# JoshuaQSH/FALCON-TTDforGNNs

Measured on NVIDIA B200. Metric: TT-EmbeddingBag rows/s fwd+bwd+SGD, higher is better.
Workload: dtype f32

## Files before the change

### falcon-ttdforgnns_b200/csrc/tt_rmma.cu

```cuda
#include <stdlib.h>

#include "common.cuh"

namespace ttg {

namespace {

constexpr int kThreads = 512;
constexpr int kWarps = kThreads / 32;
constexpr uint32_t kFull = 0xffffffffu;
constexpr int kCS = 20;

__device__ __forceinline__ uint32_t smem_u32(const void* p) { return (uint32_t)__cvta_generic_to_shared(p); }

__device__ __forceinline__ void mma_tf32(float (&c)[4], uint32_t a0, uint32_t a1, uint32_t a2, uint32_t a3,
                                         uint32_t b0, uint32_t b1) {
  asm("mma.sync.aligned.m16n8k8.row.col.f32.tf32.tf32.f32 {%0,%1,%2,%3}, {%4,%5,%6,%7}, {%8,%9}, "
      "{%0,%1,%2,%3};"
      : "+f"(c[0]), "+f"(c[1]), "+f"(c[2]), "+f"(c[3])
      : "r"(a0), "r"(a1), "r"(a2), "r"(a3), "r"(b0), "r"(b1));
}
__device__ __forceinline__ float lo_of(float x) {
  return x - __uint_as_float(__float_as_uint(x) & 0xffffe000u);
}
// ... 510 lines not shown
      const uint32_t grp = __shfl_sync(kFull, my_grp, 0);
      const uint32_t same = __ballot_sync(kFull, pos + (lane & 7) < re && my_grp == grp) & 0xffu;
      const int n = min(4, __ffs(~same) - 1);
      const bool group_ends = ((same >> n) & 1u) == 0;
      const bool more = pos + n < re;
      const uint32_t next_grp = __shfl_sync(kFull, my_grp, n);
      if (group_ends && more) prefetch_tr1<C>(a.tab, next_grp, lane);
      int i0r[4];
#pragma unroll
      for (int j = 0; j < 4; ++j) {
        const int v = __shfl_sync(kFull, my_i0, j);
        i0r[j] = (j < n) ? v : -1;
      }
      const int slot_pos = (pos - rs) & (kRing - 1);
      RM_PHASE(0);
      cp_async_wait<kRing / 4 - 1>();
      __syncwarp();
      RM_PHASE(1);
#ifdef TTG_R_TIMING
      if (pos == rs) RM_MARK(3);
#endif

      float g0[2][4];
#pragma unroll
      for (int nt = 0; nt < 2; ++nt)
#pragma unroll
        for (int e = 0; e < 4; ++e) g0[nt][e] = 0.f;
      {
        const float* pa = ring + ((slot_pos + rg) & (kRing - 1)) * RS;
        const float* pb = ring + ((slot_pos + rg + 2) & (kRing - 1)) * RS;
#pragma unroll
        for (int ks = 0; ks < 4; ++ks) {
          const float x0 = pa[xoff<C>(j0, col_k<C>(ks, 0, t))], x2 = pa[xoff<C>(j0, col_k<C>(ks, 1, t))];
          const float x1 = pb[xoff<C>(j0, col_k<C>(ks, 0, t))], x3 = pb[xoff<C>(j0, col_k<C>(ks, 1, t))];
          const uint32_t h0 = __float_as_uint(x0), h1 = __float_as_uint(x1), h2 = __float_as_uint(x2),
                         h3 = __float_as_uint(x3);
          if (TERMS == 3) {
            const uint32_t l0 = __float_as_uint(lo_of(x0)), l1 = __float_as_uint(lo_of(x1)),
                           l2 = __float_as_uint(lo_of(x2)), l3 = __float_as_uint(lo_of(x3));
#pragma unroll
            for (int nt = 0; nt < 2; ++nt) mma_tf32(g0[nt], l0, l1, l2, l3, bgh[ks][nt][0], bgh[ks][nt][1]);
#pragma unroll
            for (int nt = 0; nt < 2; ++nt) mma_tf32(g0[nt], h0, h1, h2, h3, bgl[ks][nt][0], bgl[ks][nt][1]);
          }
#pragma unroll
          for (int nt = 0; nt < 2; ++nt) mma_tf32(g0[nt], h0, h1, h2, h3, bgh[ks][nt][0], bgh[ks][nt][1]);
        }
      }
      RM_PHASE(2);
      if (group_ends && more) load_tr1_bwd<C, TERMS>(a.tab, next_grp, g, t, bgh, bgl);
      RM_PHASE(3);

#pragma unroll
      for (int ks = 0; ks < 2; ++ks) {
        const float* ce = c0s + ((i0r[2 * ks] < 0 ? a.c0_rows : i0r[2 * ks]) * 4 + t) * kCSB + g;
        const float* co = c0s + ((i0r[2 * ks + 1] < 0 ? a.c0_rows : i0r[2 * ks + 1]) * 4 + t) * kCSB + g;
        const float a0 = ce[0], a1 = ce[8], a2 = co[0], a3 = co[8];
        const uint32_t ah0 = __float_as_uint(a0), ah1 = __float_as_uint(a1), ah2 = __float_as_uint(a2),
                       ah3 = __float_as_uint(a3);
        const uint32_t al0 = __float_as_uint(lo_of(a0)), al1 = __float_as_uint(lo_of(a1)),
                       al2 = __float_as_uint(lo_of(a2)), al3 = __float_as_uint(lo_of(a3));
        const float* pe = ring + ((slot_pos + 2 * ks) & (kRing - 1)) * RS;
        const float* po = ring + ((slot_pos + 2 * ks + 1) & (kRing - 1)) * RS;
#pragma unroll
        for (int nt = 0; nt < 4; ++nt) {
          const float b0 = pe[xoff<C>(t, col_n<C>(nt, g))], b1 = po[xoff<C>(t, col_n<C>(nt, g))];
          if (TERMS == 3) {
            mma_tf32(s1[nt], al0, al1, al2, al3, __float_as_uint(b0), __float_as_uint(b1));
            mma_tf32(s1[nt], ah0, ah1, ah2, ah3, __float_as_uint(lo_of(b0)), __float_as_uint(lo_of(b1)));
          }
          mma_tf32(s1[nt], ah0, ah1, ah2, ah3, __float_as_uint(b0), __float_as_uint(b1));
        }
      }

      RM_PHASE(4);
      {
        int i0a = rg ? i0r[1] : i0r[0], i0b = rg ? i0r[3] : i0r[2];
        i0a = i0a < 0 ? a.c0_rows + warp : i0a;
        i0b = i0b < 0 ? a.c0_rows + warp : i0b;
        const int ra = i0a * 4 + j0, rb = i0b * 4 + j0;
        float* da = d0s + ra * 16;
        float* db = d0s + rb * 16;
        const int swa = d0_swizzle(ra), swb = d0_swizzle(rb);
        float* addr[8];
        float val[8];
#pragma unroll
        for (int nt = 0; nt < 2; ++nt)
#pragma unroll
          for (int e = 0; e < 2; ++e) {
            addr[4 * nt + e] = da + ((2 * t + 8 * nt + e) ^ swa);
            val[4 * nt + e] = g0[nt][e];
            addr[4 * nt + 2 + e] = db + ((2 * t + 8 * nt + e) ^ swb);
            val[4 * nt + 2 + e] = g0[nt][2 + e];
          }
        shared_add_batch<8>(addr, val);
      }

      RM_PHASE(5);
      ++chain;
      if (group_ends || chain == kChain) {
        float* dst = a.S1 + (size_t)grp * (16 * C);
#pragma unroll
        for (int nt = 0; nt < 4; ++nt) {
#pragma unroll
          for (int e = 0; e < 2; ++e) {
            const int c = col_n<C>(nt, 2 * t + e);
            if ((C % 8 == 0) || c < C) {
              float* d0 = dst + g * C + c;
              float* d1 = dst + (g + 8) * C + c;
              float v0 = s1[nt][e], v1 = s1[nt][2 + e];
              if (stored) {
                v0 += ld_dep_f32(d0);
                v1 += ld_dep_f32(d1);
              }
              *d0 = v0;
              *d1 = v1;
            }
          }
#pragma unroll
          for (int e = 0; e < 4; ++e) s1[nt][e] = 0.f;
        }
        stored = !group_ends;
        chain = 0;
      }
      __syncwarp();
      pos += n;
      RM_PHASE(6);
    }
    RM_PHASE_FLUSH;
    cp_async_wait<0>();
    __syncwarp();
  }
  }
  RM_MARK(4);
  __syncthreads();
  float* part = a.d0parts + (size_t)blockIdx.x * a.c0_rows * 64;
  for (int i = threadIdx.x; i < a.c0_rows * 64; i += kBT) part[i] = d0s[(i & ~15) + ((i & 15) ^ d0_swizzle(i >> 4))];
  RM_MARK(5);
}

constexpr int kCoresThreads = 512, kCoresWarps = kCoresThreads / 32;
constexpr int kCoresGB = 8;
constexpr int kCoresBufs = 3;
constexpr int kC2S = 24;

#ifdef TTG_R_TIMING
__device__ unsigned long long g_rc_marks[1024 * 6];
#define RC_MARK(i) \
  if (threadIdx.x == 0 && blockIdx.x < 1024) g_rc_marks[blockIdx.x * 6 + (i)] = gtime()
#else
#define RC_MARK(i)
#endif

template <int Q1, int Q2>
__global__ void __launch_bounds__(kCoresThreads, 1)
rm_cores_kernel(TTDev tt, const float* S1, const int32_t* cnt, float* __restrict__ dcore1, float* __restrict__ parts2,
                int dbg) {
  constexpr int C = Q1 * Q2, NR = 16 * Q1, IMG = 16 * C, R2 = 16, GB = kCoresGB;
  constexpr int KB = GB * Q2;
  constexpr int KSA = KB / 8;
  constexpr int MT = NR / 16;
  constexpr int NTB = KB / 8;
  constexpr int KSB = NR / 8;
  constexpr int BLK4 = GB * IMG / 4;
  static_assert(KB % 8 == 0 && NR % 16 == 0 && 2 * MT + NTB <= kCoresWarps, "tile shapes");
  extern __shared__ __align__(16) float sm[];
  const int p1 = tt.p[1], p2 = tt.p[2];
  const int nblk = (p2 + GB - 1) / GB;
  float* c2s = sm;
  float* sbuf = c2s + (size_t)nblk * KB * kC2S;
  __shared__ int32_t cnts[512 + kCoresGB];
  const int lane = threadIdx.x & 31, warp = threadIdx.x >> 5, g = lane >> 2, t = lane & 3;
  const int ti1 = blockIdx.x, table = ti1 / p1;
  const size_t h0 = (size_t)ti1 * p2;
  RC_MARK(0);
  pdl_trigger();
  {
    const float* core2 = tt.core[2] + (size_t)table * p2 * (R2 * Q2);
    constexpr int PER = kCoresThreads / (R2 * Q2);
    const int e = threadIdx.x % (R2 * Q2), k2 = e / Q2, j2 = e % Q2;
    if (threadIdx.x < PER * R2 * Q2)
      for (int i2 = threadIdx.x / (R2 * Q2); i2 < nblk * GB; i2 += PER)
        c2s[((size_t)i2 * Q2 + j2) * kC2S + k2] = (i2 < p2) ? __ldg(core2 + (size_t)i2 * (R2 * Q2) + e) : 0.f;
  }
  const bool role_a = warp < 2 * MT, role_b = !role_a && warp < 2 * MT + NTB;
  uint32_t ah[KSB][4], al[KSB][4];
  if (role_b) {
    const float* c1 = tt.core[1] + (size_t)ti1 * (NR * R2);
#pragma unroll
    for (int ks = 0; ks < KSB; ++ks) {
      const float v0 = __ldg(c1 + (t + 8 * ks) * R2 + g), v1 = __ldg(c1 + (t + 8 * ks) * R2 + g + 8);
      const float v2 = __ldg(c1 + (t + 4 + 8 * ks) * R2 + g), v3 = __ldg(c1 + (t + 4 + 8 * ks) * R2 + g + 8);
      ah[ks][0] = __float_as_uint(v0);
      ah[ks][1] = __float_as_uint(v1);
      ah[ks][2] = __float_as_uint(v2);
      ah[ks][3] = __float_as_uint(v3);
      al[ks][0] = __float_as_uint(lo_of(v0));
      al[ks][1] = __float_as_uint(lo_of(v1));
      al[ks][2] = __float_as_uint(lo_of(v2));
      al[ks][3] = __float_as_uint(lo_of(v3));
    }
  }
  RC_MARK(1);
  pdl_wait();
  RC_MARK(2);
  for (int i = threadIdx.x; i < nblk * GB; i += kCoresThreads) cnts[i] = (i < p2) ? ld_dep_s32(cnt + h0 + i) : 0;
  __syncthreads();
  RC_MARK(3);
  auto stage = [&](int blk) {
    if (blk < nblk && !(dbg & 2)) {
      float* dst = sbuf + (size_t)(blk % kCoresBufs) * (GB * IMG);
      const float* src = S1 + (h0 + (size_t)blk * GB) * IMG;
      for (int i = threadIdx.x; i < BLK4; i += kCoresThreads) {
        if (cnts[blk * GB + i / (IMG / 4)] > 0)
          cp_async16(dst + 4 * i, src + 4 * i);
        else
          *reinterpret_cast<float4*>(dst + 4 * i) = make_float4(0.f, 0.f, 0.f, 0.f);
      }
    }
    cp_async_commit();
  };
  const int mt = warp >> 1, nt = warp & 1;
  int offa[KSA][2];
#pragma unroll
  for (int ks = 0; ks < KSA; ++ks)
#pragma unroll
    for (int h = 0; h < 2; ++h) {
      const int kk = t + 4 * h + 8 * ks;
      offa[ks][h] = (kk / Q2) * IMG + (kk % Q2) + (g + 16 * mt) * Q2;
    }
  const int ntb = warp - 2 * MT;
  const int nnb = g + 8 * ntb, offb = (nnb / Q2) * IMG + (nnb % Q2) + t * Q2;
  float acc1[2][4] = {{0.f, 0.f, 0.f, 0.f}, {0.f, 0.f, 0.f, 0.f}};
  stage(0);
  stage(1);
  for (int blk = 0; blk < nblk; ++blk) {
    cp_async_wait<1>();
    __syncthreads();
#ifdef TTG_R_TIMING
    if (blk == 0) RC_MARK(4);
#endif
    stage(blk + 2);
    const float* sb = sbuf + (size_t)(blk % kCoresBufs) * (GB * IMG);
    if (dbg & 1) continue;
    if (role_a) {
      const float* cb = c2s + (size_t)blk * KB * kC2S + g + 8 * nt;
      float part[3][4] = {{0.f, 0.f, 0.f, 0.f}, {0.f, 0.f, 0.f, 0.f}, {0.f, 0.f, 0.f, 0.f}};
#pragma unroll
      for (int ks = 0; ks < KSA; ++ks) {
        const float a0 = sb[offa[ks][0]], a1 = sb[offa[ks][0] + 8 * Q2];
        const float a2 = sb[offa[ks][1]], a3 = sb[offa[ks][1] + 8 * Q2];
        const float b0 = cb[(t + 8 * ks) * kC2S], b1 = cb[(t + 4 + 8 * ks) * kC2S];
        mma_tf32(part[0], __float_as_uint(lo_of(a0)), __float_as_uint(lo_of(a1)), __float_as_uint(lo_of(a2)),
                 __float_as_uint(lo_of(a3)), __float_as_uint(b0), __float_as_uint(b1));
        mma_tf32(part[1], __float_as_uint(a0), __float_as_uint(a1), __float_as_uint(a2), __float_as_uint(a3),
                 __float_as_uint(lo_of(b0)), __float_as_uint(lo_of(b1)));
        mma_tf32(part[2], __float_as_uint(a0), __float_as_uint(a1), __float_as_uint(a2), __float_as_uint(a3),
                 __float_as_uint(b0), __float_as_uint(b1));
      }
#pragma unroll
      for (int e = 0; e < 4; ++e) {
        acc1[0][e] += part[0][e] + part[1][e];
        acc1[1][e] += part[2][e];
      }
    } else if (role_b) {
      float a_lh[2][4] = {{0.f, 0.f, 0.f, 0.f}, {0.f, 0.f, 0.f, 0.f}}, a_hl[2][4] = {{0.f, 0.f, 0.f, 0.f}, {0.f, 0.f, 0.f, 0.f}},
            a_hh[2][4] = {{0.f, 0.f, 0.f, 0.f}, {0.f, 0.f, 0.f, 0.f}};
#pragma unroll
      for (int ks = 0; ks < KSB; ++ks) {
        const float b0 = sb[offb + 8 * ks * Q2], b1 = sb[offb + (4 + 8 * ks) * Q2];
        mma_tf32(a_lh[ks & 1], al[ks][0], al[ks][1], al[ks][2], al[ks][3], __float_as_uint(b0), __float_as_uint(b1));
        mma_tf32(a_hl[ks & 1], ah[ks][0], ah[ks][1], ah[ks][2], ah[ks][3], __float_as_uint(lo_of(b0)),
                 __float_as_uint(lo_of(b1)));
        mma_tf32(a_hh[ks & 1], ah[ks][0], ah[ks][1], ah[ks][2], ah[ks][3], __float_as_uint(b0), __float_as_uint(b1));
      }
#pragma unroll
      for (int e = 0; e < 2; ++e) {
        const int nn = 2 * t + e + 8 * ntb, gi = nn / Q2, j2 = nn % Q2, i2 = blk * GB + gi;
        if (i2 < p2) {
          float* out2 = parts2 + (h0 + i2) * (R2 * Q2) + j2;
          out2[g * Q2] = ((a_lh[0][e] + a_lh[1][e]) + (a_hl[0][e] + a_hl[1][e])) + (a_hh[0][e] + a_hh[1][e]);
          out2[(g + 8) * Q2] = ((a_lh[0][2 + e] + a_lh[1][2 + e]) + (a_hl[0][2 + e] + a_hl[1][2 + e])) +
                               (a_hh[0][2 + e] + a_hh[1][2 + e]);
        }
      }
    }
  }
  cp_async_wait<0>();
  if (role_a) {
    float* out1 = dcore1 + (size_t)ti1 * (NR * R2) + (g + 16 * mt) * R2 + 2 * t + 8 * nt;
    float v[4];
#pragma unroll
    for (int e = 0; e < 4; ++e) v[e] = acc1[0][e] + acc1[1][e];
    *reinterpret_cast<float2*>(out1) = make_float2(v[0], v[1]);
    *reinterpret_cast<float2*>(out1 + 8 * R2) = make_float2(v[2], v[3]);
  }
  RC_MARK(5);
}

}

namespace {

FastDiv make_div(uint32_t d) {
  FastDiv f;
  f.d = d;
  uint32_t s = 0;
  while ((2u << s) < d) ++s;
  f.s = s;
  f.m = (uint32_t)((((uint64_t)1 << (32 + s)) + d - 1) / d);
  return f;
}

void fill_args(const TTDev& tt, const RPlan& pl, RmArgs* a) {
  memset(a, 0, sizeof(*a));
  a->skeys = pl.skeys;
  a->srow = pl.srow;
  a->base = pl.base;
  a->tab = pl.tab;
  a->core0 = tt.core[0];
  a->S1 = pl.S1;
  a->d0parts = pl.d0parts;
  a->num_groups = tt.num_tables * tt.p[1] * tt.p[2];
  a->p0 = tt.p[0];
  a->c0_rows = tt.num_tables * tt.p[0];
// ... 138 lines not shown
```

### falcon-ttdforgnns_b200/csrc/tt_tc5.cu

```cuda
#include <stdlib.h>

#include "tc5.cuh"

namespace ttg {

namespace {

using namespace tc5;

constexpr int kWorkWarps = 4;
constexpr int kThreadsR = (kWorkWarps + 2) * 32;
constexpr int kThreadsRB = (2 * kWorkWarps + 2) * 32;
constexpr int kTileRows = 32;
constexpr int kNB = 4;
constexpr int kMaxTiles = 512;
constexpr int kFwdTiles = 256;
constexpr uint32_t kFull = 0xffffffffu;

template <int Q1, int Q2>
struct RShape {
  static constexpr int C = Q1 * Q2;
  static constexpr int D = 4 * C;
  static constexpr int R1 = 16;
  static constexpr int kImg = R1 * C;
  static constexpr int kLbo = C * 16;
  static constexpr int kSlotBytes = ((2 * kImg * 4 + 128 + 255) / 256) * 256;
  static constexpr int kC0Stride = 20;
};

struct Tile {
  int32_t row0;
  int32_t n;
  int32_t group;
  int32_t flags;
};

struct RFwdArgs {
  const uint32_t* skeys;
  const int32_t* srow;
  const int32_t* base;
  const float* tab;
  const float* core0;
  float* output;
  int32_t num_groups;
  int32_t p0;
  int32_t c0_rows;
  int32_t hp;
};

__device__ int warp_lower_bound(const int32_t* base, int n, int target, int lane) {
  int lo = 0, hi = n;
  while (hi > lo) {
    const int step = (hi - lo + 31) / 32;
    const int idx = lo + lane * step;
    const bool ge = (idx >= hi) || (ld_dep_s32(base + idx) >= target);
    const uint32_t m = __ballot_sync(kFull, ge);
    if (m == 0) {
      lo = lo + 31 * step + 1;
    } else {
      const int f = __ffs(m) - 1;
      if (f == 0) {
        hi = lo;
      } else {
        const int nlo = lo + (f - 1) * step + 1;
        hi = lo + f * step;
        lo = nlo;
      }
    }
  }
  return lo;
}

__device__ int build_tiles(const int32_t* base, int& g, int& off, int g_hi, Tile* tiles, int lane,
                           int kCap = kMaxTiles) {
  int T = 0;
  while (g < g_hi && T < kCap) {
    const int gg = g + lane;
    int b0 = 0, b1 = 0;
    if (gg < g_hi) {
      b0 = ld_dep_s32(base + gg);
      b1 = ld_dep_s32(base + gg + 1);
    }
    const bool cont = (lane == 0 && off != 0);
    if (lane == 0) b0 += off;
    const int nt = (b1 - b0 + kTileRows - 1) / kTileRows;
    int incl = nt;
#pragma unroll
    for (int o = 1; o < 32; o <<= 1) {
      const int y = __shfl_up_sync(kFull, incl, o);
      if (lane >= o) incl += y;
    }
    const uint32_t fits = __ballot_sync(kFull, T + incl <= kCap);
    const int k = (fits == kFull) ? 32 : (__ffs(~fits) - 1);
    if (k == 0) {
      if (T != 0) break;
      const int b0l = __shfl_sync(kFull, b0, 0);
      for (int i = lane; i < kCap; i += 32) {
        Tile t;
        t.row0 = b0l + i * kTileRows;
        t.n = kTileRows;
        t.group = g;
        t.flags = (i == 0 && off == 0) ? 1 : 0;
        tiles[i] = t;
      }
      off += kCap * kTileRows;
      T = kCap;
      break;
    }
    if (lane < k && gg < g_hi) {
      const int pos = T + incl - nt;
      for (int i = 0; i < nt; ++i) {
        Tile t;
        t.row0 = b0 + i * kTileRows;
        t.n = min(kTileRows, b1 - t.row0);
        t.group = gg;
        t.flags = ((i == 0 && !cont) ? 1 : 0) | ((i == nt - 1) ? 2 : 0);
        tiles[pos + i] = t;
      }
    }
    T += __shfl_sync(kFull, incl, k - 1);
    g += k;
    off = 0;
    if (k < 32) break;
  }
  __syncwarp();
  return T;
}

template <int Q1, int Q2, int R2>
__global__ void __launch_bounds__(128) r_table_kernel(TTDev tt, float* __restrict__ tab, int i2_per_cta, int planes) {
  using S = RShape<Q1, Q2>;
  constexpr int C = S::C, R1 = S::R1, NF4 = S::kImg / 4;
  extern __shared__ __align__(16) float c2s[];
  pdl_trigger();
  const int ti1 = blockIdx.x;
  const int table = ti1 / tt.p[1];
  const int i2_lo = blockIdx.y * i2_per_cta;
  const int i2_n = min(i2_per_cta, tt.p[2] - i2_lo);
  const int f = threadIdx.x;
  pdl_wait();
  const float* core2 = tt.core[2] + ((size_t)table * tt.p[2] + i2_lo) * (R2 * Q2);
  for (int i = threadIdx.x; i < i2_n * R2 * Q2 / 4; i += 128)
    reinterpret_cast<float4*>(c2s)[i] = ld_dep_float4(core2 + 4 * i);
  float c1[4][R2];
  const int kc = f / C, c = f % C, j1 = c / Q2, j2 = c % Q2;
  if (f < NF4) {
    const float* core1 = tt.core[1] + (size_t)ti1 * (R1 * Q1 * R2);
#pragma unroll
    for (int kq = 0; kq < 4; ++kq)
#pragma unroll
      for (int k4 = 0; k4 < R2 / 4; ++k4) {
        const float4 v = ld_dep_float4(core1 + ((4 * kc + kq) * Q1 + j1) * R2 + 4 * k4);
        c1[kq][4 * k4 + 0] = v.x;
        c1[kq][4 * k4 + 1] = v.y;
        c1[kq][4 * k4 + 2] = v.z;
        c1[kq][4 * k4 + 3] = v.w;
      }
  }
  __syncthreads();
  if (f >= NF4) return;
  const size_t h0 = ((size_t)table * tt.p[1] + (ti1 % tt.p[1])) * tt.p[2] + i2_lo;
  for (int i = 0; i < i2_n; ++i) {
    const float* c2 = c2s + i * (R2 * Q2) + j2;
    float v[4] = {0.f, 0.f, 0.f, 0.f};
#pragma unroll
    for (int k2 = 0; k2 < R2; ++k2) {
      const float b = c2[k2 * Q2];
#pragma unroll
      for (int kq = 0; kq < 4; ++kq) v[kq] = fmaf(c1[kq][k2], b, v[kq]);
    }
    float* dst = tab + (h0 + i) * (2 * S::kImg) + 4 * f;
    *reinterpret_cast<float4*>(dst) = make_float4(v[0], v[1], v[2], v[3]);
    if (planes == 2)
      *reinterpret_cast<float4*>(dst + S::kImg) =
          make_float4(tf32_lo(v[0]), tf32_lo(v[1]), tf32_lo(v[2]), tf32_lo(v[3]));
  }
}

struct RSmem {
  uint64_t a_full[2], d_full[2], b_full[kNB], b_empty[kNB];
  uint32_t tmem_base;
  int32_t range[2];
  int32_t ntiles;
  int32_t more;
};

template <int Q1, int Q2, int TERMS>
__global__ void __launch_bounds__(kThreadsR, 4) r_fwd_kernel(RFwdArgs a) {
  using S = RShape<Q1, Q2>;
  constexpr int C = S::C, D = S::D;
  extern __shared__ __align__(1024) unsigned char smem[];
  unsigned char* bring = smem;
  Tile* tiles = reinterpret_cast<Tile*>(bring + kNB * S::kSlotBytes);
  float* rowbuf = reinterpret_cast<float*>(tiles + kFwdTiles);
  RSmem* sm = reinterpret_cast<RSmem*>(rowbuf + kWorkWarps * 8 * D);

  const int tid = threadIdx.x, warp = tid >> 5, lane = tid & 31;
  pdl_trigger();
  if (tid == 0) {
    mbar_init(&sm->a_full[0], kWorkWarps);
    mbar_init(&sm->a_full[1], kWorkWarps);
    mbar_init(&sm->d_full[0], 1);
    mbar_init(&sm->d_full[1], 1);
    for (int i = 0; i < kNB; ++i) {
      mbar_init(&sm->b_full[i], 1);
      mbar_init(&sm->b_empty[i], 1);
    }
    mbar_init_fence();
  }
  for (int i = tid; i < kNB * S::kSlotBytes / 4; i += kThreadsR) reinterpret_cast<float*>(bring)[i] = 0.f;
  fence_proxy_async();
  if (warp == 0) tmem_alloc(&sm->tmem_base, 128);
  pdl_wait();
  if (warp < 2) {
    const int total = ld_dep_s32(a.base + a.num_groups);
    const int chunk = (total + (int)gridDim.x - 1) / (int)gridDim.x;
    const int target = ((int)blockIdx.x + warp) * chunk;
    int g = warp_lower_bound(a.base, a.num_groups + 1, target, lane);
    if (g > a.num_groups || ((int)blockIdx.x + warp) >= (int)gridDim.x) g = a.num_groups;
    if (blockIdx.x == 0 && warp == 0) g = 0;
    if (lane == 0) sm->range[warp] = g;
  }
  fence_before();
  __syncthreads();
  fence_after();
  const uint32_t tbase = sm->tmem_base;
  const int g_hi = sm->range[1];
  int g_next = sm->range[0], g_off = 0;
  uint32_t gt = 0;
  uint32_t gq = 0;

  while (true) {
    if (warp == 5) {
      const int T = build_tiles(a.base, g_next, g_off, g_hi, tiles, lane, kFwdTiles);
      if (lane == 0) {
        sm->ntiles = T;
        sm->more = (g_next < g_hi) ? 1 : 0;
      }
    }
    __syncthreads();
    const int T = sm->ntiles;
    const int more = sm->more;
    if (warp < kWorkWarps) {
      const int r = lane >> 2, j0 = lane & 3, slot = warp * 8 + r;
      const uint32_t lane_base = tbase + ((uint32_t)(warp * 32) << 16);
      float* myrows = rowbuf + warp * 8 * D;
      uint32_t key_n = 0, key_nn = 0;
      int32_t srow_c = 0, srow_n = 0, srow_nn = 0;
      auto load_keys = [&](int t, uint32_t& key, int32_t& sr) {
        key = 0;
        sr = 0;
        if (t < T) {
          const Tile tl = tiles[t];
          if (slot < tl.n) {
            key = ld_dep_u32(a.skeys + tl.row0 + slot);
            sr = ld_dep_s32(a.srow + tl.row0 + slot);
          }
        }
      };
      auto fill = [&](int t, uint32_t key) {
        const Tile tl = tiles[t];
        const uint32_t s = (gt + (uint32_t)t) & 1u;
        if (warp * 8 < tl.n) {
          uint32_t hi[16], lo[16];
          if (slot < tl.n) {
            const uint32_t i0 = key % (uint32_t)a.p0;
            const uint32_t tbl = (a.c0_rows == a.p0) ? 0u : (key / (uint32_t)a.p0) / (uint32_t)a.hp;
            const float4* src = reinterpret_cast<const float4*>(a.core0) + ((size_t)(tbl * a.p0 + i0) * 4 + j0) * 4;
#pragma unroll
            for (int q = 0; q < 4; ++q) {
              const float4 v = __ldg(src + q);
              hi[4 * q + 0] = __float_as_uint(v.x);
              hi[4 * q + 1] = __float_as_uint(v.y);
              hi[4 * q + 2] = __float_as_uint(v.z);
              hi[4 * q + 3] = __float_as_uint(v.w);
            }
          } else {
#pragma unroll
            for (int i = 0; i < 16; ++i) hi[i] = 0u;
          }
          st16(lane_base + s * 32, hi);
          if (TERMS == 3) {
#pragma unroll
            for (int i = 0; i < 16; ++i) lo[i] = __float_as_uint(tf32_lo(__uint_as_float(hi[i])));
            st16(lane_base + s * 32 + 16, lo);
          }
          wait_st();
        }
        fence_before();
        __syncwarp();
        if (lane == 0) mbar_arrive(&sm->a_full[s]);
      };
      auto epilogue = [&](int t, int32_t sr) {
        const Tile tl = tiles[t];
        const uint32_t u = gt + (uint32_t)t, s = u & 1u;
        mbar_wait(&sm->d_full[s], (u >> 1) & 1u);
        fence_after();
        if (warp * 8 < tl.n) {
          uint32_t v[32];
          ld32(lane_base + 64 + s * 32, v);
          wait_ld();
          if constexpr (C % 4 == 0) {
#pragma unroll
            for (int i = 0; i < C / 4; ++i) {
              const int pos = j0 * (C / 4) + (i ^ (lane & 7));
              *reinterpret_cast<float4*>(myrows + r * D + 4 * pos) =
                  make_float4(__uint_as_float(v[4 * i]), __uint_as_float(v[4 * i + 1]),
                              __uint_as_float(v[4 * i + 2]), __uint_as_float(v[4 * i + 3]));
            }
          } else {
#pragma unroll
            for (int c = 0; c < C; ++c) myrows[r * D + j0 * C + c] = __uint_as_float(v[c]);
          }
          __syncwarp();
          const int nrows = min(8, tl.n - warp * 8);
#pragma unroll
          for (int rr = 0; rr < 8; ++rr) {
            const int32_t orow = __shfl_sync(kFull, sr, 4 * rr);
            if (rr < nrows && lane < D / 4) {
              float4 val;
              if constexpr (C % 4 == 0) {
                const int jj = lane / (C / 4), i = lane % (C / 4);
// ... 711 lines not shown
      float v[2] = {0.f, 0.f};
#pragma unroll
      for (int w = 0; w < 2; ++w) {
        const int x = tid + w * 256;
        if (x < NGA * R2 * Q2) {
          const int u = x / (R2 * Q2), e = x % (R2 * Q2), i2 = trip * NGA + u;
          if (i2 < tt.p[2]) v[w] = __ldg(core2 + (size_t)i2 * (R2 * Q2) + e);
        }
      }
      return make_float2(v[0], v[1]);
    };
    auto store_c2 = [&](int buf, float2 v) {
#pragma unroll
      for (int w = 0; w < 2; ++w) {
        const int x = tid + w * 256;
        if (x < NGA * R2 * Q2) {
          const int u = x / (R2 * Q2), e = x % (R2 * Q2);
          c2t[((size_t)buf * NGA + u) * (R2 * Q2) + (e % Q2) * R2 + e / Q2] = w ? v.y : v.x;
        }
      }
    };
    float acc[R2];
#pragma unroll
    for (int i = 0; i < R2; ++i) acc[i] = 0.f;
    stage(0, 0);
    store_c2(0, load_c2(0));
    for (int trip = 0; trip < ntrips; ++trip) {
      const int buf = trip & 1;
      float2 c2n = make_float2(0.f, 0.f);
      if (trip + 1 < ntrips) {
        stage(trip + 1, buf ^ 1);
        c2n = load_c2(trip + 1);
        cp_async_wait<1>();
      } else {
        cp_async_wait<0>();
      }
      __syncthreads();
      if (worker) {
        const float* st = s1s + ((size_t)buf * NGA + grp) * IMG + (kj / Q1) * C + (kj % Q1) * Q2;
        const float* ct = c2t + ((size_t)buf * NGA + grp) * (R2 * Q2);
#pragma unroll
        for (int j2 = 0; j2 < Q2; ++j2) {
          const float sv = st[j2];
#pragma unroll
          for (int k4 = 0; k4 < R2 / 4; ++k4) {
            const float4 cv = *reinterpret_cast<const float4*>(ct + j2 * R2 + 4 * k4);
            acc[4 * k4 + 0] = fmaf(sv, cv.x, acc[4 * k4 + 0]);
            acc[4 * k4 + 1] = fmaf(sv, cv.y, acc[4 * k4 + 1]);
            acc[4 * k4 + 2] = fmaf(sv, cv.z, acc[4 * k4 + 2]);
            acc[4 * k4 + 3] = fmaf(sv, cv.w, acc[4 * k4 + 3]);
          }
        }
      }
      __syncthreads();
      if (trip + 1 < ntrips) store_c2(buf ^ 1, c2n);
    }
    if (worker) {
#pragma unroll
      for (int k4 = 0; k4 < R2 / 4; ++k4)
        *reinterpret_cast<float4*>(red + ((size_t)grp * NKJ + kj) * R2 + 4 * k4) =
            make_float4(acc[4 * k4], acc[4 * k4 + 1], acc[4 * k4 + 2], acc[4 * k4 + 3]);
    }
    __syncthreads();
    for (int o = tid; o < NKJ * R2 / 4; o += 256) {
      float4 v = reinterpret_cast<const float4*>(red)[o];
#pragma unroll
      for (int g = 1; g < NGA; ++g) {
        const float4 w = reinterpret_cast<const float4*>(red + (size_t)g * NKJ * R2)[o];
        v.x += w.x;
        v.y += w.y;
        v.z += w.z;
        v.w += w.w;
      }
      reinterpret_cast<float4*>(dcore1 + (size_t)ti1 * (NKJ * R2))[o] = v;
    }
  } else {
    constexpr int TPG = R2 / 4 * Q2;
    const int ti2 = blockIdx.x - nb1, table = ti2 / tt.p[2], i2 = ti2 % tt.p[2];
    const float* core1 = tt.core[1] + (size_t)table * tt.p[1] * (NKJ * R2);
    float* s1s = sh;
    float* red = sh + kBufB;
    for (int i = tid; i < tt.p[1]; i += 256) cnts[i] = cnt[((size_t)table * tt.p[1] + i) * tt.p[2] + i2];
    __syncthreads();
    const int grp = tid / TPG, k2q = (tid % TPG) / Q2, j2 = tid % Q2;
    const bool worker = tid < NGB * TPG;
    const int ntrips = (tt.p[1] + NGB - 1) / NGB;
    auto stage = [&](int trip, int buf) {
      for (int i = tid; i < NGB * (IMG / 4); i += 256) {
        const int u = i / (IMG / 4), e = i % (IMG / 4), i1 = trip * NGB + u;
        float* dst = s1s + ((size_t)buf * NGB + u) * IMG + 4 * e;
        if (i1 < tt.p[1] && cnts[i1] > 0)
          cp_async16(dst, S1 + (((size_t)table * tt.p[1] + i1) * tt.p[2] + i2) * IMG + 4 * e);
        else
          *reinterpret_cast<float4*>(dst) = make_float4(0.f, 0.f, 0.f, 0.f);
      }
      cp_async_commit();
    };
    float acc[4] = {0.f, 0.f, 0.f, 0.f};
    stage(0, 0);
    for (int trip = 0; trip < ntrips; ++trip) {
      const int buf = trip & 1;
      if (trip + 1 < ntrips) {
        stage(trip + 1, buf ^ 1);
        cp_async_wait<1>();
      } else {
        cp_async_wait<0>();
      }
      __syncthreads();
      const int i1 = trip * NGB + grp;
      if (worker && i1 < tt.p[1] && cnts[i1] > 0) {
        const float* st = s1s + ((size_t)buf * NGB + grp) * IMG + j2;
        const float4* c1 = reinterpret_cast<const float4*>(core1 + (size_t)i1 * (NKJ * R2)) + k2q;
#pragma unroll 8
        for (int t = 0; t < NKJ; ++t) {
          const float4 cv = __ldg(c1 + t * (R2 / 4));
          const float sv = st[(t / Q1) * C + (t % Q1) * Q2];
          acc[0] = fmaf(cv.x, sv, acc[0]);
          acc[1] = fmaf(cv.y, sv, acc[1]);
          acc[2] = fmaf(cv.z, sv, acc[2]);
          acc[3] = fmaf(cv.w, sv, acc[3]);
        }
      }
      __syncthreads();
    }
    if (worker) {
#pragma unroll
      for (int e = 0; e < 4; ++e) red[grp * (R2 * Q2) + (4 * k2q + e) * Q2 + j2] = acc[e];
    }
    __syncthreads();
    if (tid < R2 * Q2) {
      float v = 0.f;
#pragma unroll
      for (int g = 0; g < NGB; ++g) v += red[g * (R2 * Q2) + tid];
      dcore2[(size_t)ti2 * (R2 * Q2) + tid] = v;
    }
  }
}

}

namespace {

template <int Q1, int Q2>
size_t r_fwd_smem(int c0_rows) {
  using S = RShape<Q1, Q2>;
  (void)c0_rows;
  return (size_t)kNB * S::kSlotBytes + sizeof(Tile) * kFwdTiles + sizeof(float) * kWorkWarps * 8 * S::D +
         sizeof(RSmem) + 64;
}

template <int Q1, int Q2>
int r_table_launch(const TTDev& tt, const RPlan& pl, int planes, cudaStream_t stream) {
  constexpr int R2 = 16;
  const int nb = tt.num_tables * tt.p[1];
  int split = (int)ceil_div(4 * kNumSMs, nb);
  if (split < 1) split = 1;
  int per = (int)ceil_div(tt.p[2], split);
  if (per < 4) per = 4;
  if (per > 128) per = 128;
  split = (int)ceil_div(tt.p[2], per);
  const size_t smem = sizeof(float) * (size_t)per * R2 * Q2;
  auto kern = r_table_kernel<Q1, Q2, R2>;
  TTG_ENSURE_SMEM(kern, sizeof(float) * 128 * R2 * Q2);
  prof_begin(K_TABLE, stream);
  TTG_CUDA(launch_pdl<2>(kern, dim3(nb, split), dim3(128), smem, stream, tt, pl.tab, per, planes));
  prof_end(K_TABLE, stream);
  TTG_LAUNCH_CHECK();
  return TTG_OK;
}

template <int Q1, int Q2, int TERMS>
int r_fwd_launch(const TTDev& tt, int64_t nnz, const RPlan& pl, float* output, cudaStream_t stream) {
  RFwdArgs a;
  a.skeys = pl.skeys;
  a.srow = pl.srow;
  a.base = pl.base;
  a.tab = pl.tab;
  a.core0 = tt.core[0];
  a.output = output;
  a.num_groups = tt.num_tables * tt.p[1] * tt.p[2];
  a.p0 = tt.p[0];
  a.c0_rows = tt.num_tables * tt.p[0];
  a.hp = tt.p[1] * tt.p[2];
  const size_t smem = r_fwd_smem<Q1, Q2>(a.c0_rows);
  auto kern = r_fwd_kernel<Q1, Q2, TERMS>;
  TTG_ENSURE_SMEM(kern, smem);
  static const int cps = [] { const char* v = getenv("TTG_R_CPS"); return v ? atoi(v) : 4; }();
  int64_t grid = (int64_t)kNumSMs * cps;
  if (grid * 64 > nnz) grid = ceil_div(nnz, 64);
  prof_begin(K_FWD, stream);
  TTG_CUDA(launch_pdl(kern, dim3((unsigned)grid), dim3(kThreadsR), smem, stream, a));
  prof_end(K_FWD, stream);
  TTG_LAUNCH_CHECK();
  return TTG_OK;
}

template <int Q1, int Q2>
size_t r_bwd_smem(int c0_rows) {
  using S = RShape<Q1, Q2>;
  return (size_t)2 * 2 * kTileRows * 256 + (size_t)kNBG * 2 * 2048 + (size_t)kNB * S::kSlotBytes +
         sizeof(float) * (2 * kTileRows * S::D + kTileRows * 64 + 2 * 4 * 16 * 32) + sizeof(Tile) * kMaxTiles +
         sizeof(float) * (size_t)c0_rows * 64 + sizeof(int32_t) * ((c0_rows + 3) & ~3) + sizeof(RBSmem) + 64;
}

template <int Q1, int Q2>
int r_cores_launch(const TTDev& tt, const RPlan& pl, float* const* dcore, cudaStream_t stream) {
  const int nb = tt.num_tables * (tt.p[1] + tt.p[2]);
  prof_begin(K_BWD_CORES, stream);
  TTG_CUDA(launch_pdl(r_cores_kernel<Q1, Q2, 16>, dim3(nb), dim3(256), 0, stream, tt, (const float*)pl.S1, pl.cnt,
                      dcore[1], dcore[2]));
  prof_end(K_BWD_CORES, stream);
  TTG_LAUNCH_CHECK();
  return TTG_OK;
}

template <int Q1, int Q2, int TERMS>
int r_bwd_launch(const TTDev& tt, int64_t nnz, const RPlan& pl, const float* d_output, float* const* dcore,
                 int* nparts, cudaStream_t stream) {
  RBwdArgs a;
  a.skeys = pl.skeys;
  a.srow = pl.srow;
  a.base = pl.base;
  a.tab = pl.tab;
  a.core0 = tt.core[0];
  a.d_output = d_output;
  a.S1 = pl.S1;
  a.d0parts = pl.d0parts;
  a.num_groups = tt.num_tables * tt.p[1] * tt.p[2];
  a.p0 = tt.p[0];
  a.c0_rows = tt.num_tables * tt.p[0];
  a.hp = tt.p[1] * tt.p[2];
  const size_t smem = r_bwd_smem<Q1, Q2>(a.c0_rows);
  auto kern = r_bwd_kernel<Q1, Q2, TERMS>;
  TTG_ENSURE_SMEM(kern, smem);
  int64_t grid = kNumSMs;
  if (grid * 64 > nnz) grid = ceil_div(nnz, 64);
  *nparts = (int)grid;
  prof_begin(K_BWD_ROWS, stream);
  TTG_CUDA(launch_pdl(kern, dim3((unsigned)grid), dim3(kThreadsRB), smem, stream, a));
  prof_end(K_BWD_ROWS, stream);
  TTG_LAUNCH_CHECK();
  return r_cores_launch<Q1, Q2>(tt, pl, dcore, stream);
}

struct REntry {
  int q1, q2;
  int (*table)(const TTDev&, const RPlan&, int, cudaStream_t);
  int (*fwd[2])(const TTDev&, int64_t, const RPlan&, float*, cudaStream_t);
  int (*bwd[2])(const TTDev&, int64_t, const RPlan&, const float*, float* const*, int*, cudaStream_t);
  size_t (*fwd_smem)(int);
  size_t (*bwd_smem)(int);
};

#define TTG_R_SHAPE(Q1, Q2)                                                                          \
  {                                                                                                  \
    Q1, Q2, r_table_launch<Q1, Q2>, {r_fwd_launch<Q1, Q2, 3>, r_fwd_launch<Q1, Q2, 1>},              \
        {r_bwd_launch<Q1, Q2, 3>, r_bwd_launch<Q1, Q2, 1>}, r_fwd_smem<Q1, Q2>, r_bwd_smem<Q1, Q2>  \
  }

const REntry kREntries[] = {
    TTG_R_SHAPE(5, 5),
    TTG_R_SHAPE(4, 8),
};

const REntry* find_r(const TTDev& tt) {
  if (tt.T != 3 || tt.q[0] != 4 || tt.r[1] != 16 || tt.r[2] != 16) return nullptr;
  if (tt.p[1] > 512 || tt.p[2] > 512) return nullptr;
  for (const REntry& e : kREntries)
    if (e.q1 == tt.q[1] && e.q2 == tt.q[2]) {
      if (e.fwd_smem(tt.num_tables * tt.p[0]) > 220 * 1024 || e.bwd_smem(tt.num_tables * tt.p[0]) > 220 * 1024)
        return nullptr;
      return &e;
    }
  return nullptr;
}

}

#ifdef TTG_R_TIMING
extern "C" void ttg_r_timing(long long* out, int reset) {
  if (reset) {
    long long z[16] = {0};
    cudaMemcpyToSymbol(g_rtime, z, sizeof(z));
  } else {
    cudaMemcpyFromSymbol(out, g_rtime, sizeof(long long) * 16);
  }
}
#endif

bool r_supported(const TTDev& tt) { return find_r(tt) != nullptr; }

size_t r_table_floats(const TTDev& tt) {
  return (size_t)tt.num_tables * tt.p[1] * tt.p[2] * 2 * 16 * (tt.q[1] * tt.q[2]);
}

int r_table(const TTDev& tt, const RPlan& pl, int planes, cudaStream_t stream) {
  const REntry* e = find_r(tt);
  if (!e) return TTG_ENOTSUP;
  return e->table(tt, pl, planes, stream);
}

int r_backward(const TTDev& tt, int64_t nnz, const RPlan& pl, const float* d_output, float* const* dcore,
               int32_t optim, float lr, float eps, float* const* state, bool tf32, cudaStream_t stream) {
  const REntry* e = find_r(tt);
  if (!e) return TTG_ENOTSUP;
  int nparts = 0;
  int rc = e->bwd[tf32 ? 1 : 0](tt, nnz, pl, d_output, dcore, &nparts, stream);
  if (rc != TTG_OK) return rc;
  return mma_finalize_parts(tt, pl.d0parts, nparts, nullptr, 0, dcore, optim, lr, eps, state, stream);
}

int r_cores(const TTDev& tt, const RPlan& pl, float* const* dcore, cudaStream_t stream) {
  if (!find_r(tt)) return TTG_ENOTSUP;
  if (tt.q[1] == 5 && tt.q[2] == 5) return r_cores_launch<5, 5>(tt, pl, dcore, stream);
  if (tt.q[1] == 4 && tt.q[2] == 8) return r_cores_launch<4, 8>(tt, pl, dcore, stream);
  return TTG_ENOTSUP;
}

// ... 8 lines not shown
```

Before: 1.509 billion.

## Transpose core2 smem layout, split table kernel into i2 slots, remap core warp roles

The table-precompute kernel now stores core2 in shared memory transposed and padded, so each thread reads its R2 coefficients as float4 vectors instead of strided scalars. It launches two thread slots per image element that split the i2 loop, and sizes the grid split from occupancy rather than a fixed multiplier. Separately, the cores kernel permutes warp-to-role assignment for the MT=5,NTB=5 shape, probably to balance roles across SM sub-partitions. The cost is a more complex scatter on load and a different grid shape that may change tail behaviour.

Result: no change. 1.509 billion, median of 6 (+0.0%).

```diff
diff --git a/falcon-ttdforgnns_b200/csrc/tt_rmma.cu b/falcon-ttdforgnns_b200/csrc/tt_rmma.cu
--- a/falcon-ttdforgnns_b200/csrc/tt_rmma.cu
+++ b/falcon-ttdforgnns_b200/csrc/tt_rmma.cu
@@ -686,6 +686,15 @@
 #define RC_MARK(i)
 #endif
 
+template <int MT, int NTB>
+__device__ __forceinline__ int cores_role(int warp) {
+  if (MT == 5 && NTB == 5) {
+    constexpr unsigned long long kSlots = 0xF9876543E210DCBAull;
+    return (int)((kSlots >> (4 * warp)) & 15);
+  }
+  return warp;
+}
+
 template <int Q1, int Q2>
 __global__ void __launch_bounds__(kCoresThreads, 1)
 rm_cores_kernel(TTDev tt, const float* S1, const int32_t* cnt, float* __restrict__ dcore1, float* __restrict__ parts2,
@@ -704,7 +713,8 @@
   float* c2s = sm;
   float* sbuf = c2s + (size_t)nblk * KB * kC2S;
   __shared__ int32_t cnts[512 + kCoresGB];
-  const int lane = threadIdx.x & 31, warp = threadIdx.x >> 5, g = lane >> 2, t = lane & 3;
+  const int lane = threadIdx.x & 31, g = lane >> 2, t = lane & 3;
+  const int warp = cores_role<MT, NTB>(threadIdx.x >> 5);
   const int ti1 = blockIdx.x, table = ti1 / p1;
   const size_t h0 = (size_t)ti1 * p2;
   RC_MARK(0);
diff --git a/falcon-ttdforgnns_b200/csrc/tt_tc5.cu b/falcon-ttdforgnns_b200/csrc/tt_tc5.cu
--- a/falcon-ttdforgnns_b200/csrc/tt_tc5.cu
+++ b/falcon-ttdforgnns_b200/csrc/tt_tc5.cu
@@ -127,24 +127,29 @@
   return T;
 }
 
+constexpr int kTabSlots = 2;
+template <int Q1, int Q2>
+constexpr int tab_threads() { return RShape<Q1, Q2>::kImg / 4 * kTabSlots; }
+template <int R2>
+constexpr int tab_c2_stride() { return R2 + 4; }
+
 template <int Q1, int Q2, int R2>
-__global__ void __launch_bounds__(128) r_table_kernel(TTDev tt, float* __restrict__ tab, int i2_per_cta, int planes) {
+__global__ void __launch_bounds__(tab_threads<Q1, Q2>()) r_table_kernel(TTDev tt, float* __restrict__ tab, int i2_per_cta,
+                                                                       int planes) {
   using S = RShape<Q1, Q2>;
-  constexpr int C = S::C, R1 = S::R1, NF4 = S::kImg / 4;
+  constexpr int C = S::C, R1 = S::R1, NF4 = S::kImg / 4, NT = tab_threads<Q1, Q2>(), CS = tab_c2_stride<R2>();
+  constexpr int kBatch = 2;
   extern __shared__ __align__(16) float c2s[];
   pdl_trigger();
   const int ti1 = blockIdx.x;
   const int table = ti1 / tt.p[1];
   const int i2_lo = blockIdx.y * i2_per_cta;
   const int i2_n = min(i2_per_cta, tt.p[2] - i2_lo);
-  const int f = threadIdx.x;
+  const int f = threadIdx.x % NF4, slot = threadIdx.x / NF4;
   pdl_wait();
-  const float* core2 = tt.core[2] + ((size_t)table * tt.p[2] + i2_lo) * (R2 * Q2);
-  for (int i = threadIdx.x; i < i2_n * R2 * Q2 / 4; i += 128)
-    reinterpret_cast<float4*>(c2s)[i] = ld_dep_float4(core2 + 4 * i);
   float c1[4][R2];
   const int kc = f / C, c = f % C, j1 = c / Q2, j2 = c % Q2;
-  if (f < NF4) {
+  {
     const float* core1 = tt.core[1] + (size_t)ti1 * (R1 * Q1 * R2);
 #pragma unroll
     for (int kq = 0; kq < 4; ++kq)
@@ -157,17 +162,37 @@
         c1[kq][4 * k4 + 3] = v.w;
       }
   }
+  const float* core2 = tt.core[2] + ((size_t)table * tt.p[2] + i2_lo) * (R2 * Q2);
+  const int n4 = i2_n * R2 * Q2 / 4;
+  for (int b = threadIdx.x; b < n4; b += kBatch * NT) {
+    float4 v[kBatch];
+#pragma unroll
+    for (int u = 0; u < kBatch; ++u)
+      if (b + u * NT < n4) v[u] = ld_dep_float4(core2 + 4 * (b + u * NT));
+#pragma unroll
+    for (int u = 0; u < kBatch; ++u)
+      if (b + u * NT < n4) {
+        const float w[4] = {v[u].x, v[u].y, v[u].z, v[u].w};
+#pragma unroll
+        for (int l = 0; l < 4; ++l) {
+          const int e = 4 * (b + u * NT) + l, i = e / (R2 * Q2), k2 = (e / Q2) % R2;
+          c2s[(i * Q2 + e % Q2) * CS + k2] = w[l];
+        }
+      }
+  }
   __syncthreads();
-  if (f >= NF4) return;
   const size_t h0 = ((size_t)table * tt.p[1] + (ti1 % tt.p[1])) * tt.p[2] + i2_lo;
-  for (int i = 0; i < i2_n; ++i) {
-    const float* c2 = c2s + i * (R2 * Q2) + j2;
+  for (int i = slot; i < i2_n; i += kTabSlots) {
+    const float4* c2 = reinterpret_cast<const float4*>(c2s + (i * Q2 + j2) * CS);
     float v[4] = {0.f, 0.f, 0.f, 0.f};
 #pragma unroll
-    for (int k2 = 0; k2 < R2; ++k2) {
-      const float b = c2[k2 * Q2];
-#pragma unroll
-      for (int kq = 0; kq < 4; ++kq) v[kq] = fmaf(c1[kq][k2], b, v[kq]);
+    for (int k4 = 0; k4 < R2 / 4; ++k4) {
+      const float4 w = c2[k4];
+      const float b[4] = {w.x, w.y, w.z, w.w};
+#pragma unroll
+      for (int l = 0; l < 4; ++l)
+#pragma unroll
+        for (int kq = 0; kq < 4; ++kq) v[kq] = fmaf(c1[kq][4 * k4 + l], b[l], v[kq]);
     }
     float* dst = tab + (h0 + i) * (2 * S::kImg) + 4 * f;
     *reinterpret_cast<float4*>(dst) = make_float4(v[0], v[1], v[2], v[3]);
@@ -1185,18 +1210,26 @@
 template <int Q1, int Q2>
 int r_table_launch(const TTDev& tt, const RPlan& pl, int planes, cudaStream_t stream) {
   constexpr int R2 = 16;
+  constexpr int NT = tab_threads<Q1, Q2>(), kMaxPer = 128;
   const int nb = tt.num_tables * tt.p[1];
-  int split = (int)ceil_div(4 * kNumSMs, nb);
+  auto kern = r_table_kernel<Q1, Q2, R2>;
+  TTG_ENSURE_SMEM(kern, sizeof(float) * kMaxPer * Q2 * tab_c2_stride<R2>());
+  static const int resident = [&] {
+    int n = 0;
+    if (cudaOccupancyMaxActiveBlocksPerMultiprocessor(&n, kern, NT, sizeof(float) * 32 * Q2 * tab_c2_stride<R2>()) !=
+            cudaSuccess || n < 1)
+      n = 1;
+    return n;
+  }();
+  int split = (resident * kNumSMs) / nb;
   if (split < 1) split = 1;
   int per = (int)ceil_div(tt.p[2], split);
-  if (per < 4) per = 4;
-  if (per > 128) per = 128;
+  if (per < 2 * kTabSlots) per = 2 * kTabSlots;
+  if (per > kMaxPer) per = kMaxPer;
   split = (int)ceil_div(tt.p[2], per);
-  const size_t smem = sizeof(float) * (size_t)per * R2 * Q2;
-  auto kern = r_table_kernel<Q1, Q2, R2>;
-  TTG_ENSURE_SMEM(kern, sizeof(float) * 128 * R2 * Q2);
+  const size_t smem = sizeof(float) * (size_t)per * Q2 * tab_c2_stride<R2>();
   prof_begin(K_TABLE, stream);
-  TTG_CUDA(launch_pdl<2>(kern, dim3(nb, split), dim3(128), smem, stream, tt, pl.tab, per, planes));
+  TTG_CUDA(launch_pdl<2>(kern, dim3(nb, split), dim3(NT), smem, stream, tt, pl.tab, per, planes));
   prof_end(K_TABLE, stream);
   TTG_LAUNCH_CHECK();
   return TTG_OK;
```
